# YonghaoHe/LFD-A-Light-and-Fast-Detector

Hardware: NVIDIA H100
Metric: images/sec WIDERFACE-S inference 1280x720 batch=8 per GPU bf16 (higher is better)
Workload: dtype bf16

## Files before the change

### lfd-a-light-and-fast-detector_b200/csrc/conv_umma.cu

```cuda
#include <stdlib.h>

#include <type_traits>

#include "conv_common.cuh"
#include "ptx.cuh"

namespace lfd {

static constexpr int kProdThreads = 128;
static constexpr int kConsumerThreads = 256;
static constexpr int kConvThreads = kConsumerThreads + kProdThreads;

#define LFD_LAMBDA_INLINE __attribute__((always_inline))

#ifdef LFD_B200_TRACE
#define LFD_TRACE(role, idx, slot) \
    do { if (p.trace && blockIdx.x == 0 && (idx) < 32) p.trace[((role) * 32 + (idx)) * 4 + (slot)] = clock64(); } while (0)
#define LFD_TRACE_EPI(tr, idx, slot) \
    do { if ((tr) && blockIdx.x == 0 && (idx) < 16) (tr)[(idx) * 8 + (slot)] = clock64(); } while (0)
#else
#define LFD_TRACE(role, idx, slot) ((void)0)
#define LFD_TRACE_EPI(tr, idx, slot) ((void)0)
#endif

// ... 359 lines not shown
                        store_tile<MODE, COUT, F16>(e, acc3, COUT, bias2, false, false, nullptr, &p.tm_out3, nullptr, c0, c1, n, v0, v1,
                                                    &res_bar[wg], store_count, res_count);
                }
            }
        }
        if (e.wtid == 0) bulk_wait_all();
    } else {
        asm volatile("setmaxnreg.dec.sync.aligned.u32 56;");
        const int ptid = tid - kConsumerThreads;
        if (MODE == MODE_STEM) {
            const bool u8 = p.input_format == 1;
            const int plane = p.H * p.W;
            int rel[kStemPerThread];
            int prc[kStemPerThread];
#pragma unroll
            for (int j = 0; j < kStemPerThread; ++j) {
                const int q = min(ptid + j * kProdThreads, kStemPix - 1);
                const int r = q / kStemCols, c = q - r * kStemCols;
                prc[j] = (r << 8) | c;
                rel[j] = u8 ? (r * p.W + c) * 3 : r * p.W + c;
            }
            const bool last_ok = ptid + (kStemPerThread - 1) * kProdThreads < kStemPix;
            uint32_t raw[kStemPerThread][3];
            uint32_t okmask = 0;
            auto fetch = [&](int tile) LFD_LAMBDA_INLINE {
                const int n = fast_div(tile, p.magic_tpi), t = tile - n * p.tiles_per_img;
                const int ty = fast_div(t, p.magic_tx);
                const int iy0 = 2 * ty * 16 - 1, ix0 = 2 * (t - ty * p.tiles_x) * 8 - 1;
                const bool interior = iy0 >= 0 && ix0 >= 0 && iy0 + kStemRows <= p.H && ix0 + kStemCols <= p.W;
                okmask = 0;
                if (u8) {
                    const uint8_t* img = reinterpret_cast<const uint8_t*>(p.in_raw) + (size_t)n * plane * 3;
                    const uint8_t* org = img + ((ptrdiff_t)iy0 * p.W + ix0) * 3;
#pragma unroll
                    for (int j = 0; j < kStemPerThread; ++j) {
                        if (j == kStemPerThread - 1 && !last_ok) break;
                        const uint8_t* src = org + rel[j];
                        bool ok = true;
                        if (!interior) {
                            const int y = iy0 + (prc[j] >> 8), x = ix0 + (prc[j] & 255);
                            ok = (unsigned)y < (unsigned)p.H && (unsigned)x < (unsigned)p.W;
                            if (!ok) src = img;
                        }
                        okmask |= (ok ? 1u : 0u) << j;
                        raw[j][0] = __ldg(src); raw[j][1] = __ldg(src + 1); raw[j][2] = __ldg(src + 2);
                    }
                } else {
                    const float* img = reinterpret_cast<const float*>(p.in_raw) + (size_t)n * plane * 3;
                    const float* org = img + (ptrdiff_t)iy0 * p.W + ix0;
#pragma unroll
                    for (int j = 0; j < kStemPerThread; ++j) {
                        if (j == kStemPerThread - 1 && !last_ok) break;
                        const float* src = org + rel[j];
                        bool ok = true;
                        if (!interior) {
                            const int y = iy0 + (prc[j] >> 8), x = ix0 + (prc[j] & 255);
                            ok = (unsigned)y < (unsigned)p.H && (unsigned)x < (unsigned)p.W;
                            if (!ok) src = img;
                        }
                        okmask |= (ok ? 1u : 0u) << j;
                        raw[j][0] = __float_as_uint(__ldg(src)); raw[j][1] = __float_as_uint(__ldg(src + plane));
                        raw[j][2] = __float_as_uint(__ldg(src + 2 * plane));
                    }
                }
            };
            uint32_t it = 0;
            pdl_wait();
            if ((int)blockIdx.x < p.num_tiles) fetch(blockIdx.x);
            for (int tile = blockIdx.x; tile < p.num_tiles; tile += gridDim.x, ++it) {
                const uint32_t s = it % SA, ph = (it / SA) & 1;
                if (ptid == 0) LFD_TRACE(0, it, 0);
                mbar_wait(&empty[s], ph ^ 1);
                if (ptid == 0) LFD_TRACE(0, it, 1);
                const uint32_t dst0 = smem_u32(ring) + s * p.stage_bytes + ptid * 8;
#pragma unroll
                for (int j = 0; j < kStemPerThread; ++j) {
                    if (j == kStemPerThread - 1 && !last_ok) break;
                    float f[3];
#pragma unroll
                    for (int k = 0; k < 3; ++k) {
                        f[k] = u8 ? ((float)raw[j][k] - 127.5f) * (1.0f / 127.5f) : __uint_as_float(raw[j][k]);
                        if (!((okmask >> j) & 1u)) f[k] = 0.f;
                    }
                    const uint32_t lo = pack2<F16>(f[0], f[1]), hi = pack2<F16>(f[2], 0.f);
                    asm volatile("st.shared.v2.b32 [%0], {%1, %2};" ::"r"(dst0 + j * (kProdThreads * 8)), "r"(lo), "r"(hi) : "memory");
                }
                fence_proxy_async_smem();
                mbar_arrive(&full[s]);
                if (ptid == 0) LFD_TRACE(0, it, 2);
                if (tile + (int)gridDim.x < p.num_tiles) fetch(tile + gridDim.x);
                if (ptid == 0) LFD_TRACE(0, it, 3);
            }
        } else {
        const int ch = ptid & (cpc - 1);
        const int px0 = ptid >> p.log2_cpc;
        const int pstep = kProd >> p.log2_cpc;
        const uint32_t ch_dst = ch * p.lbo_a;
        const int my_cnt = (p.n_px - px0 + pstep - 1) / pstep;
        uint32_t it = 0;
        pdl_wait();
        for (int tile = blockIdx.x; tile < p.num_tiles; tile += gridDim.x) {
            const int n = fast_div(tile, p.magic_tpi);
            const int t = tile - n * p.tiles_per_img;
            int iy0 = 0, ix0 = 0;
            if (MODE == MODE_FLAT) ix0 = t * 128;
            else {
                const int ty = fast_div(t, p.magic_tx);
                int oy0 = ty * 16, ox0 = (t - ty * p.tiles_x) * 8;
                iy0 = (MODE == MODE_3X3S1) ? oy0 : 2 * oy0;
                ix0 = (MODE == MODE_3X3S1) ? ox0 : 2 * ox0;
            }
            const __nv_bfloat16* img = p.in + (size_t)n * HW * p.Cin + ch * 8;
            constexpr int kDyMin = (MODE == MODE_1X1S2) ? 0 : -1, kDxMin = kDyMin;
            constexpr int kDyMax = (MODE == MODE_3X3S1) ? 16 : ((MODE == MODE_3X3S2) ? 31 : 30);
            constexpr int kDxMax = (MODE == MODE_3X3S1) ? 8 : ((MODE == MODE_3X3S2) ? 15 : 14);
            const bool interior = MODE == MODE_FLAT ? (ix0 + 128 <= HW)
                                                    : (iy0 + kDyMin >= 0 && ix0 + kDxMin >= 0 && iy0 + kDyMax < p.H && ix0 + kDxMax < p.W);
            const __nv_bfloat16* org = img + (ptrdiff_t)(MODE == MODE_FLAT ? ix0 : (iy0 + kDyMin) * p.W + ix0 + kDxMin) * p.Cin;
            for (int cc = 0; cc < n_cc; ++cc, ++it) {
                const uint32_t s = it % SA, ph = (it / SA) & 1;
                if (ptid == 0) LFD_TRACE(0, it, 0);
                mbar_wait(&empty[s], ph ^ 1);
                if (ptid == 0) LFD_TRACE(0, it, 1);
                const uint32_t a_base = smem_u32(ring) + s * p.stage_bytes;
                if (!p.b_resident && ptid == 0) {
                    mbar_arrive_expect_tx(&full[s], p.b_slice_bytes);
                    bulk_g2s(a_base + p.a_stage_bytes, reinterpret_cast<const uint8_t*>(p.w) + (size_t)cc * p.b_slice_bytes,
                             p.b_slice_bytes, &full[s]);
                }
                const __nv_bfloat16* src_cc = img + cc * p.Cc;
                const uint32_t dst_cc = a_base + ch_dst;
                if (MODE == MODE_FLAT) {
                    if (interior) {
                        const __nv_bfloat16* src = org + cc * p.Cc + (size_t)px0 * p.Cin;
                        const size_t sstep = (size_t)pstep * p.Cin;
                        uint32_t dst = dst_cc + px0 * 16;
#pragma unroll 4
                        for (int pxi = px0; pxi < 128; pxi += pstep, src += sstep, dst += pstep * 16) cp_async16_full(dst, src);
                    } else {
#pragma unroll 4
                        for (int pxi = px0; pxi < 128; pxi += pstep) {
                            const int q = ix0 + pxi;
                            const bool ok = q < HW;
                            cp_async16(dst_cc + pxi * 16, src_cc + (ok ? q : 0) * p.Cin, ok);
                        }
                    }
                } else if (interior) {
                    const uint8_t* src = reinterpret_cast<const uint8_t*>(org + cc * p.Cc);
                    const PxEntry* tp = table + px0;
#pragma unroll 4
                    for (int k = 0; k < my_cnt; ++k, tp += pstep) {
                        const uint2 pe = *reinterpret_cast<const uint2*>(tp);
                        cp_async16_full(dst_cc + pe.y, src + pe.x);
                    }
                } else {
#pragma unroll 2
                    for (int pxi = px0; pxi < p.n_px; pxi += pstep) {
                        const PxDelta pd = delta[pxi];
                        const int y = iy0 + pd.dy, x = ix0 + pd.dx;
                        const bool ok = ((unsigned)y < (unsigned)p.H) && ((unsigned)x < (unsigned)p.W);
                        cp_async16(dst_cc + table[pxi].dst_off, src_cc + (ok ? (y * p.W + x) : 0) * p.Cin, ok);
                    }
                }
                cp_async_mbar_arrive(&full[s]);
                if (ptid == 0) LFD_TRACE(0, it, 2);
            }
        }
        cp_async_wait_all();
        }
    }
    LFD_TL_END(p.tl);
}

static constexpr int kS4Rows = 67, kS4Cols = 36, kS4Pix = kS4Rows * kS4Cols;
static constexpr int kS4RowBytes = kS4Cols * 8;
static constexpr int kS4PatchBytes = kS4Pix * 8;
static constexpr int kS4PerThread = (kS4Pix + kProdThreads - 1) / kProdThreads;
static constexpr int kS4Batch = 5;
static constexpr int kS4Groups = kS4Rows * 10;
static constexpr int kS4GroupsPerThread = (kS4Groups + kProdThreads - 1) / kProdThreads;
static constexpr int kS4GroupBatch = 3;
static constexpr int kS4PatchOverrun = 768;
LFD_DEVINL constexpr int s4_slot(int a, int b) {
    return ((a & 1) ? ((b & 1) ? 0 : 147) : ((b & 1) ? 291 : 446)) + (a >> 1) * 9 + (b >> 1);
}
static constexpr int kS4Lbo = 599 * 16;
static constexpr int kS4Bar = 0;
static constexpr int kS4Shift = 256;
static constexpr int kS4Staging = 2048;
static constexpr int kS4W0 = kS4Staging + 2 * 8192;
static constexpr int kS4W1 = kS4W0 + 6144;
static constexpr int kS4W2 = kS4W1 + 8192;
static constexpr int kS4W3 = kS4W2 + 73728;
static constexpr int kS4Planes = kS4W3 + 8192;
static constexpr int kS4Ring = kS4Planes + 8 * kS4Lbo;
static constexpr int kS4Smem = kS4Ring + 2 * kS4PatchBytes + kS4PatchOverrun;
static constexpr int kS4WBytes = kS4Planes - kS4W0;
static_assert(kS4Smem <= 227 * 1024, "stem4 shared memory");

LFD_DEVINL void s4_block(int i, int& a0, int& b0, bool& packed) {
    packed = i == 8 || i == 13;
    a0 = packed ? 32 : 8 * (i < 8 ? i >> 1 : i - 9);
    b0 = i < 8 ? 1 + 8 * (i & 1) : (i == 8 ? 1 : 0);
}
LFD_DEVINL void s4_run(int num_tiles, int& t0, int& t1) {
    t0 = (int)((uint64_t)blockIdx.x * (uint32_t)num_tiles / gridDim.x);
    t1 = (int)((uint64_t)(blockIdx.x + 1) * (uint32_t)num_tiles / gridDim.x);
}

LFD_DEVINL void consumers_bar_sync() { asm volatile("bar.sync 3, 256;" ::: "memory"); }

template <bool F16>
__global__ void __launch_bounds__(kConvThreads, 1) stem4_kernel(const __grid_constant__ UmmaConvParams p) {
    extern __shared__ __align__(1024) uint8_t smem[];
    uint64_t* full = reinterpret_cast<uint64_t*>(smem + kS4Bar);
    uint64_t* empty = full + 2;
    uint64_t* wbar = empty + 2;
    uint64_t* res_bar = wbar + 1;
    float* shifts = reinterpret_cast<float*>(smem + kS4Shift);
    pdl_launch_dependents();
    LFD_TL_BEGIN(p.tl);
    const int tid = threadIdx.x;
    const int warp = tid >> 5;
    const int lane = tid & 31;
    if (tid == 0) {
        for (int i = 0; i < 2; ++i) {
            mbar_init(&full[i], kProdThreads);
            mbar_init(&empty[i], kConsumerThreads / 32);
        }
        mbar_init(wbar, 1);
        mbar_init(&res_bar[0], 1);
        mbar_init(&res_bar[1], 1);
        fence_mbar_init();
    }
    if (tid < 256) {
        const int k = tid >> 6;
        const float* s = k == 0 ? p.shift : (k == 1 ? p.shift2 : (k == 2 ? p.shift_s2 : p.shift_s3));
        shifts[tid] = s ? round16<F16>(s[tid & 63]) : 0.f;
    }
    __syncthreads();

    if (warp < kConsumerThreads / 32) {
        asm volatile("setmaxnreg.inc.sync.aligned.u32 224;");
        const int wg = warp >> 2;
        if (tid == 0) {
            mbar_arrive_expect_tx(wbar, kS4WBytes);
            auto load_w = [&](uint32_t dst, const __nv_bfloat16* src, uint32_t bytes) LFD_LAMBDA_INLINE {
                for (uint32_t off = 0; off < bytes; off += 32768)
                    bulk_g2s(smem_u32(smem) + dst + off, reinterpret_cast<const uint8_t*>(src) + off, bytes - off < 32768 ? bytes - off : 32768, wbar);
            };
            load_w(kS4W0, p.w, kS4W1 - kS4W0);
            load_w(kS4W1, p.w2, kS4W2 - kS4W1);
            load_w(kS4W2, p.w_s2, kS4W3 - kS4W2);
            load_w(kS4W3, p.w_s3, kS4Planes - kS4W3);
        }
        pdl_wait();
        mbar_wait(wbar, 0);

        EpiCtx e;
        e.stg_bytes = 8192u;
        e.nbuf = 1;
        e.stg = smem_u32(smem + kS4Staging) + (uint32_t)wg * 8192u;
        e.r0 = (warp & 3) * 16 + (lane >> 2);
        e.tq = lane & 3;
        e.wtid = tid & 127;
        e.wg = wg;
        e.lane = lane;
#ifdef LFD_B200_TRACE
        e.tr = p.trace && e.wtid == 0 ? p.trace + (3 * 32 + wg) * 4 : nullptr;
#endif
        const float* sh0 = shifts;
        const float* sh1 = shifts + 64;
        const float* sh2 = shifts + 128;
        const float* sh3 = shifts + 192;
        const uint32_t planes = smem_u32(smem + kS4Planes);
        const uint64_t adesc_stem = wgmma_desc(0, 16, 2 * kS4RowBytes);
        const uint64_t adesc_row = wgmma_desc(0, 16, 8 * 16);
        const uint64_t b0desc = wgmma_desc(smem_u32(smem + kS4W0), 64 * 16, 128);
        const uint64_t b1desc = wgmma_desc(smem_u32(smem + kS4W1), 64 * 16, 128);
        const uint64_t b2desc = wgmma_desc(smem_u32(smem + kS4W2), 64 * 16, 128);
        const uint64_t b3desc = wgmma_desc(smem_u32(smem + kS4W3), 64 * 16, 128);
        const uint64_t adesc_pl = wgmma_desc(planes + (uint32_t)wg * 8u * 144u, kS4Lbo, 144);
        const int brow = 2 * (warp & 3), bcol = lane >> 2;
        const int sh = (lane >> 3) & 1, sc = lane & 7;

        int tile0, tile1;
        s4_run(p.num_tiles, tile0, tile1);
        uint32_t store_count = 0, res_count = 0;
        for (int tile = tile0, lt = 0; tile < tile1; ++tile, ++lt) {
            const uint32_t s = lt & 1, ph = (lt >> 1) & 1;
            const int n = fast_div(tile, p.magic_tpi);
            const int t = tile - n * p.tiles_per_img;
            const int ty = fast_div(t, p.magic_tx);
            const int tx = t - ty * p.tiles_x;
            const int oy0 = ty * 16, ox0 = tx * 8;
            const bool inherit = tile > tile0 && tx > 0, pass_on = tile + 1 < tile1 && tx + 1 < p.tiles_x;
            if (e.wtid == 0) LFD_TRACE(1 + wg, lt, 0);
            mbar_wait(&full[s], ph);
            if (e.wtid == 0) LFD_TRACE(1 + wg, lt, 1);
            fence_proxy_async_smem();
            const uint32_t patch = smem_u32(smem + kS4Ring) + s * kS4PatchBytes;

            const int nblk = inherit ? 9 : 14, half = (nblk + 1) >> 1;
            const int first = wg ? half : 0, cnt = wg ? nblk - half : half;
#pragma unroll 1
            for (int kp = 0; kp < (cnt + 1) >> 1; ++kp) {
                int blk[2] = {first + 2 * kp, first + min(2 * kp + 1, cnt - 1)};
                float c0[2][32];
                wgmma_fence_regs<32>(c0[0]);
                wgmma_fence_regs<32>(c0[1]);
                wgmma_fence();
#pragma unroll
                for (int q = 0; q < 2; ++q) {
                    int a0, b0;
                    bool packed;
                    s4_block(blk[q], a0, b0, packed);
                    const uint32_t boff = (uint32_t)(a0 * 2 * kS4RowBytes + b0 * 16);
                    const uint64_t ad = (packed ? adesc_row : adesc_stem) + ((patch + boff) >> 4);
#pragma unroll
                    for (int kh = 0; kh < 3; ++kh)
                        wgmma_ss<64, F16>(c0[q], ad + (uint32_t)(kh * kS4RowBytes / 16), b0desc + (uint32_t)(kh * 2 * 64 * 16 / 16), kh != 0);
                }
                wgmma_commit();
                wgmma_wait<0>();
                wgmma_fence_regs<32>(c0[0]);
                wgmma_fence_regs<32>(c0[1]);
                uint32_t a1[2][16];
#pragma unroll
                for (int q = 0; q < 2; ++q)
#pragma unroll
                    for (int kk = 0; kk < 4; ++kk) {
                        const int c = 16 * kk + 2 * e.tq;
#pragma unroll
                        for (int r = 0; r < 4; ++r) {
                            const float x0 = c0[q][8 * kk + 2 * r] + sh0[c + 8 * (r >> 1)], x1 = c0[q][8 * kk + 2 * r + 1] + sh0[c + 8 * (r >> 1) + 1];
                            a1[q][4 * kk + r] = p.relu ? pack2_relu<F16>(x0, x1) : pack2<F16>(x0, x1);
                        }
                    }
                float c1[2][32];
                wgmma_fence_regs<32>(c1[0]);
                wgmma_fence_regs<32>(c1[1]);
                wgmma_fence();
                tail_mma<64, 64, F16>(c1[0], a1[0], b1desc);
                tail_mma<64, 64, F16>(c1[1], a1[1], b1desc);
                wgmma_commit();
                wgmma_wait<0>();
                wgmma_fence_regs<32>(c1[0]);
                wgmma_fence_regs<32>(c1[1]);
                float2 bv[8];
#pragma unroll
                for (int j = 0; j < 8; ++j) bv[j] = *reinterpret_cast<const float2*>(sh1 + 8 * j + 2 * e.tq);
#pragma unroll
                for (int q = 0; q < 2; ++q) {
                    int a0, b0;
                    bool packed;
                    s4_block(blk[q], a0, b0, packed);
                    if (packed && (warp & 3)) continue;
                    uint32_t v[8][2];
#pragma unroll
                    for (int h = 0; h < 2; ++h) {
                        const int a = packed ? a0 : a0 + brow + h, b = b0 + bcol + (packed ? 8 * h : 0);
                        const int y1 = 2 * oy0 - 1 + a, x1 = 2 * ox0 - 1 + b;
                        const bool in = (unsigned)y1 < (unsigned)p.H1 && (unsigned)x1 < (unsigned)p.W1;
#pragma unroll
                        for (int j = 0; j < 8; ++j) {
                            const float x0 = c1[q][4 * j + 2 * h] + bv[j].x, x1v = c1[q][4 * j + 2 * h + 1] + bv[j].y;
                            const uint32_t w = p.relu2 ? pack2_relu<F16>(x0, x1v) : pack2<F16>(x0, x1v);
                            v[j][h] = in ? w : 0u;
                        }
                    }
                    const int a = packed ? a0 : a0 + brow + sh, b = b0 + sc + (packed ? 8 * sh : 0);
                    const uint32_t addr = planes + (uint32_t)s4_slot(a, b) * 16u + (uint32_t)(lane >> 4) * kS4Lbo;
#pragma unroll
                    for (int k = 0; k < 4; ++k)
                        stmatrix_x4(addr + (uint32_t)(2 * k * kS4Lbo), v[2 * k][0], v[2 * k][1], v[2 * k + 1][0], v[2 * k + 1][1]);
                }
            }
            __syncwarp();
            if (lane == 0) mbar_arrive(&empty[s]);
            if (e.wtid == 0) LFD_TRACE(1 + wg, lt, 2);
            fence_proxy_async_smem();
            consumers_bar_sync();
            if (e.wtid == 0) LFD_TRACE(1 + wg, lt, 3);

            float acc[32];
            wgmma_fence_regs<32>(acc);
            wgmma_fence();
#pragma unroll
            for (int k16 = 0; k16 < 4; ++k16)
#pragma unroll
                for (int tap = 0; tap < 9; ++tap)
                    wgmma_ss<64, F16>(acc, adesc_pl + (uint32_t)(k16 * 2 * kS4Lbo / 16 + s4_slot(tap / 3, tap % 3)),
                                      b2desc + (uint32_t)((tap * 8 + 2 * k16) * 64 * 16 / 16), (k16 | tap) != 0);
            wgmma_commit();
            wgmma_wait<0>();
            wgmma_fence_regs<32>(acc);
            consumers_bar_sync();
            if (pass_on) {
                const int rs = lane >> 3, a = 16 * wg + brow + (rs & 1) + 8 * (rs >> 1);
                const uint32_t src = planes + (uint32_t)(lane & 7) * kS4Lbo + (uint32_t)s4_slot(a, 16) * 16u;
                sts128(src - 8u * 16u, lds128(src));
                if (wg == 1 && brow == 0 && lane < 8) {
                    const uint32_t src32 = planes + (uint32_t)lane * kS4Lbo + (uint32_t)s4_slot(32, 16) * 16u;
                    sts128(src32 - 8u * 16u, lds128(src32));
                }
                __syncwarp();
            }
#ifdef LFD_B200_TRACE
            if (e.wtid == 0 && p.trace && blockIdx.x == 0 && lt < 16) p.trace[(3 * 32 + wg + 2 * lt) * 4 + 3] = clock64();
#endif

            uint32_t a2[16];
#pragma unroll
            for (int kk = 0; kk < 4; ++kk) {
                const int c = 16 * kk + 2 * e.tq;
#pragma unroll
                for (int r = 0; r < 4; ++r) {
                    const float x0 = acc[8 * kk + 2 * r] + sh2[c + 8 * (r >> 1)], x1 = acc[8 * kk + 2 * r + 1] + sh2[c + 8 * (r >> 1) + 1];
                    a2[4 * kk + r] = p.relu_s2 ? pack2_relu<F16>(x0, x1) : pack2<F16>(x0, x1);
                }
            }
            float acc2[32];
            wgmma_fence_regs<32>(acc2);
            wgmma_fence();
            tail_mma<64, 64, F16>(acc2, a2, b3desc);
            wgmma_commit();
            wgmma_wait<0>();
            wgmma_fence_regs<32>(acc2);
            store_tile<MODE_3X3S2, 64, F16>(e, acc2, 64, sh3, (bool)p.relu_s3, false, nullptr, &p.tm_out, &p.tm_res, ox0, oy0 + wg * 8, n,
                                            true, true, &res_bar[wg], store_count, res_count);
        }
        if (e.wtid == 0) bulk_wait_all();
    } else {
        asm volatile("setmaxnreg.dec.sync.aligned.u32 56;");
        const int ptid = tid - kConsumerThreads;
        const bool u8 = p.input_format == 1;
        const int plane = p.H * p.W;
        pdl_wait();
        int tile0, tile1;
        s4_run(p.num_tiles, tile0, tile1);
        for (int tile = tile0, lt = 0; tile < tile1; ++tile, ++lt) {
            const uint32_t s = lt & 1, ph = (lt >> 1) & 1;
            const int n = fast_div(tile, p.magic_tpi), t = tile - n * p.tiles_per_img;
            const int ty = fast_div(t, p.magic_tx);
            const int iy0 = 4 * 16 * ty - 3, ix0 = 4 * 8 * (t - ty * p.tiles_x) - 3;
            const bool interior = iy0 >= 0 && ix0 >= 0 && iy0 + kS4Rows <= p.H && ix0 + kS4Cols <= p.W;
            if (ptid == 0) LFD_TRACE(0, lt, 0);
            mbar_wait(&empty[s], ph ^ 1);
            if (ptid == 0) LFD_TRACE(0, lt, 1);
            const uint32_t dst0 = smem_u32(smem + kS4Ring) + s * kS4PatchBytes;
            if (p.in_words) {
#pragma unroll 1
                for (int j0 = 0; j0 < kS4GroupsPerThread; j0 += kS4GroupBatch) {
                    uint32_t wd[kS4GroupBatch][3];
                    bool ok[kS4GroupBatch];
#pragma unroll
                    for (int j = 0; j < kS4GroupBatch; ++j) {
                        const int q = ptid + (j0 + j) * kProdThreads;
                        const int r = q / 10, g = q - r * 10;
                        const int y = iy0 + r, x = ix0 - 1 + 4 * g;
                        ok[j] = q < kS4Groups && (unsigned)y < (unsigned)p.H && (unsigned)x < (unsigned)p.W;
                        const uint32_t* src = reinterpret_cast<const uint32_t*>(reinterpret_cast<const uint8_t*>(p.in_raw) +
                                                                                ((ptrdiff_t)n * plane + (ptrdiff_t)y * p.W + x) * 3);
#pragma unroll
                        for (int k = 0; k < 3; ++k) wd[j][k] = ok[j] ? __ldg(src + k) : 0u;
                    }
#pragma unroll
                    for (int j = 0; j < kS4GroupBatch; ++j) {
                        const int q = ptid + (j0 + j) * kProdThreads;
                        if (q >= kS4Groups) break;
                        const int r = q / 10, g = q - r * 10;
                        uint32_t px[4][2];
#pragma unroll
                        for (int k = 0; k < 4; ++k) {
                            float f[3];
#pragma unroll
                            for (int c = 0; c < 3; ++c) {
                                const uint32_t byte = (wd[j][(3 * k + c) >> 2] >> (8 * ((3 * k + c) & 3))) & 0xffu;
                                f[c] = ok[j] ? ((float)byte - 127.5f) * (1.0f / 127.5f) : 0.f;
                            }
                            px[k][0] = pack2<F16>(f[0], f[1]);
                            px[k][1] = pack2<F16>(f[2], 0.f);
                        }
                        const uint32_t d = dst0 + (uint32_t)(r * kS4RowBytes + 32 * g);
                        if (g > 0) asm volatile("st.shared.v2.b32 [%0], {%1, %2};" ::"r"(d - 8u), "r"(px[0][0]), "r"(px[0][1]) : "memory");
                        if (g < 9) {
                            asm volatile("st.shared.v4.b32 [%0], {%1, %2, %3, %4};" ::"r"(d), "r"(px[1][0]), "r"(px[1][1]), "r"(px[2][0]),
                                         "r"(px[2][1]) : "memory");
                            asm volatile("st.shared.v2.b32 [%0], {%1, %2};" ::"r"(d + 16u), "r"(px[3][0]), "r"(px[3][1]) : "memory");
                        }
                    }
                }
            } else {
#pragma unroll 1
                for (int j0 = 0; j0 < kS4PerThread; j0 += kS4Batch) {
                    uint32_t raw[kS4Batch][3];
                    bool ok[kS4Batch];
#pragma unroll
                    for (int j = 0; j < kS4Batch; ++j) {
                        const int q = ptid + (j0 + j) * kProdThreads;
                        const int r = q / kS4Cols, c = q - r * kS4Cols;
                        const int y = iy0 + r, x = ix0 + c;
                        ok[j] = q < kS4Pix && (interior || ((unsigned)y < (unsigned)p.H && (unsigned)x < (unsigned)p.W));
                        const ptrdiff_t pix = ok[j] ? (ptrdiff_t)n * plane + (ptrdiff_t)y * p.W + x : 0;
                        if (u8) {
                            const uint8_t* src = reinterpret_cast<const uint8_t*>(p.in_raw) + pix * 3;
                            raw[j][0] = __ldg(src); raw[j][1] = __ldg(src + 1); raw[j][2] = __ldg(src + 2);
                        } else {
                            const float* src = reinterpret_cast<const float*>(p.in_raw) + (ok[j] ? (ptrdiff_t)n * 2 * plane + pix : 0);
                            raw[j][0] = __float_as_uint(__ldg(src)); raw[j][1] = __float_as_uint(__ldg(src + plane));
                            raw[j][2] = __float_as_uint(__ldg(src + 2 * plane));
                        }
                    }
#pragma unroll
                    for (int j = 0; j < kS4Batch; ++j) {
                        const int q = ptid + (j0 + j) * kProdThreads;
                        if (q >= kS4Pix) break;
                        float f[3];
#pragma unroll
                        for (int k = 0; k < 3; ++k) {
                            f[k] = u8 ? ((float)raw[j][k] - 127.5f) * (1.0f / 127.5f) : __uint_as_float(raw[j][k]);
                            if (!ok[j]) f[k] = 0.f;
                        }
                        const uint32_t lo = pack2<F16>(f[0], f[1]), hi = pack2<F16>(f[2], 0.f);
                        asm volatile("st.shared.v2.b32 [%0], {%1, %2};" ::"r"(dst0 + q * 8), "r"(lo), "r"(hi) : "memory");
                    }
                }
            }
            fence_proxy_async_smem();
            mbar_arrive(&full[s]);
            if (ptid == 0) LFD_TRACE(0, lt, 2);
        }
    }
    LFD_TL_END(p.tl);
}

static int configure_with(const ConvGeom& g, int num_sms, int nbuf, UmmaConvParams* out, size_t* smem_bytes, int* grid) {
    UmmaConvParams p;
    memset(&p, 0, sizeof(p));
    p.stg_nbuf = nbuf;
    int mode;
    if (g.stem) {
        if (g.ksize != 3 || g.stride != 2 || g.Cin != 16) return -1;
        mode = MODE_STEM;
    } else if (g.ksize == 1 && g.stride == 1) mode = MODE_FLAT;
    else if (g.ksize == 3 && g.stride == 1) mode = MODE_3X3S1;
    else if (g.ksize == 3 && g.stride == 2) mode = MODE_3X3S2;
    else if (g.ksize == 1 && g.stride == 2) mode = MODE_1X1S2;
    else return -1;
    if (g.Cin % 16 || (g.Cout != 16 && g.Cout != 32 && g.Cout != 64 && g.Cout != 128)) return -1;
    if ((mode == MODE_3X3S1 || mode == MODE_3X3S2) && g.Cout < 32) return -1;
    p.mode = mode;
    p.N = g.N; p.H = g.H; p.W = g.W; p.Cin = g.Cin; p.Ho = g.Ho; p.Wo = g.Wo; p.Cout = g.Cout;
    const int taps = g.stem ? 3 : g.ksize * g.ksize;
    int px_slots;
    if (mode == MODE_FLAT) {
        p.tiles_x = 0; p.tiles_per_img = (g.Ho * g.Wo + 127) / 128;
        p.n_px = 128; px_slots = 128; p.sbo_a = 128;
    } else {
        p.tiles_x = (g.Wo + 7) / 8;
        p.tiles_per_img = p.tiles_x * ((g.Ho + 15) / 16);
        if (mode == MODE_3X3S1) { p.n_px = 180; px_slots = 180; p.sbo_a = 160; }
        else if (mode == MODE_3X3S2) { p.n_px = 561; px_slots = 594; p.sbo_a = 144; }
        else { p.n_px = 128; px_slots = 128; p.sbo_a = 128; }
    }
    const int plane_slots = px_slots | 1;
    p.lbo_a = plane_slots * 16;
    if (mode == MODE_STEM) { p.lbo_a = 16; p.sbo_a = 2 * kStemRowBytes; }
    p.num_tiles = p.tiles_per_img * g.N;
    if (p.num_tiles >= (1 << 24) || p.tiles_per_img >= (1 << 16)) return -5;
    p.magic_tpi = ((1ull << 40) + p.tiles_per_img - 1) / p.tiles_per_img;
    p.magic_tx = p.tiles_x ? ((1ull << 40) + p.tiles_x - 1) / p.tiles_x : 0;
    const int Cf = g.tail_cout > 0 ? g.tail_cout : g.Cout;
    if (g.ds_cout && (mode != MODE_3X3S2 || g.tail_cout || g.ds_cout != g.Cout)) return -6;
    if (g.tail_cout && (g.tail_cout % 16 || g.tail_cout > 128 || g.tail_cout < 16)) return -4;
    const size_t staging = (size_t)nbuf * 128 * Cf * 2;
    size_t hoff = kSmemTableOff;
    p.smem_table_off = (uint32_t)hoff;
    if (mode != MODE_FLAT && mode != MODE_STEM) hoff += ((size_t)p.n_px * 10 + 127) & ~(size_t)127;
    p.smem_bias_off = (uint32_t)hoff; hoff += ((size_t)g.Cout * 4 + 15) & ~(size_t)15;
    p.smem_bias2_off = (uint32_t)hoff; hoff += ((size_t)(g.tail_cout + g.ds_cout) * 4 + 15) & ~(size_t)15;
    p.smem_staging_off = (uint32_t)((hoff + 1023) & ~(size_t)1023);
    const size_t fixed = p.smem_staging_off + staging;
    const size_t w2_bytes = g.tail_cout ? ((size_t)g.Cout * g.tail_cout * 2 + 127) & ~(size_t)127
                                        : (g.ds_cout ? ((size_t)g.Cin * g.ds_cout * 2 + 127) & ~(size_t)127 : 0);
    const size_t post = w2_bytes;
    const size_t budget = 224 * 1024 - post;
    const size_t w_total = (size_t)taps * g.Cin * g.Cout * 2;
    const int cands[3] = {64, 32, 16};
    int best_cc = 0, best_res = 0, best_st = 0;
    auto a_bytes = [&](int cc) -> size_t {
        if (mode == MODE_STEM) return kStemPatchBytes;
        return (((size_t)plane_slots * (cc / 8) * 16) + 127) & ~(size_t)127;
    };
    auto stages_for = [&](int cc, int resident) -> int {
        if (g.Cin % cc) return 0;
        const size_t b_slice = (size_t)taps * cc * g.Cout * 2;
        const size_t stage = a_bytes(cc) + (resident ? 0 : b_slice);
        if (fixed + (resident ? w_total : 0) + 2 * stage > budget) return 0;
        int st = (int)((budget - fixed - (resident ? w_total : 0)) / stage);
        if (st > kMaxStages) st = kMaxStages;
        if (st > 4 && stage >= 8192) st = 4;
        return st;
    };
    static const int force_cc = getenv("LFD_B200_FORCE_CC") ? atoi(getenv("LFD_B200_FORCE_CC")) : 0;
    if (force_cc && mode == MODE_3X3S2) {
        int st = stages_for(force_cc, 1);
        if (st >= 2) { best_cc = force_cc; best_res = 1; best_st = st; }
    }
    for (int pass = 0; pass < 3 && !best_cc; ++pass)
        for (int ci = 0; ci < 3 && !best_cc; ++ci) {
            const int want = pass == 0 ? 3 : 2;
            if (pass < 2 && cands[ci] < 32) continue;
            int st = stages_for(cands[ci], 1);
            if (st >= want) { best_cc = cands[ci]; best_res = 1; best_st = st; }
        }
    if (!best_cc || (best_st < 3 && best_cc < 32)) {
        for (int want = 4; want >= 2; --want) {
            bool found = false;
            for (int ci = 0; ci < 3 && !found; ++ci) {
                int st = stages_for(cands[ci], 0);
                if (st >= want && (!best_cc || st > best_st)) { best_cc = cands[ci]; best_res = 0; best_st = st; found = true; }
            }
            if (found) break;
        }
    }
    if (!best_cc) return -2;
    p.Cc = best_cc; p.b_resident = best_res; p.stages = best_st;
    p.a_stage_bytes = (uint32_t)a_bytes(best_cc);
    p.b_slice_bytes = (uint32_t)((size_t)taps * best_cc * g.Cout * 2);
    p.stage_bytes = p.a_stage_bytes + (best_res ? 0 : p.b_slice_bytes);
    p.w_total_bytes = (uint32_t)w_total;
    p.smem_w_off = (uint32_t)fixed;
    p.smem_ring_off = (uint32_t)(fixed + (best_res ? w_total : 0));
    auto ilog2 = [](int v) { int l = 0; while ((1 << l) < v) ++l; return l; };
    p.log2_cpc = ilog2(p.Cc / 8);
    p.Cf = Cf;
    p.Cout2 = g.tail_cout;
    p.Cout3 = g.ds_cout;
    p.log2_cpr = ilog2(Cf / 8);
    if ((1 << p.log2_cpr) != Cf / 8) return -3;
    size_t off = p.smem_ring_off + (size_t)p.stages * p.stage_bytes;
    p.smem_w2_off = (uint32_t)off; off += w2_bytes;
    *smem_bytes = off;
    *grid = p.num_tiles < num_sms ? p.num_tiles : num_sms;
    *out = p;
    return 0;
}

static int configure_stem4(const ConvGeom& g, int num_sms, UmmaConvParams* out, size_t* smem_bytes, int* grid) {
    if (g.Cin != 3 || g.ksize != 3 || g.stride != 2 || g.Cout != 64 || g.tail_cout != 64 || g.ds_cout) return -1;
    UmmaConvParams p;
    memset(&p, 0, sizeof(p));
    p.mode = MODE_STEM4;
    p.N = g.N; p.H = g.H; p.W = g.W; p.Cin = 3; p.Cout = 64; p.Cout2 = 64; p.Cf = 64;
    p.H1 = (g.H - 1) / 2 + 1; p.W1 = (g.W - 1) / 2 + 1;
    p.Ho = (p.H1 - 1) / 2 + 1; p.Wo = (p.W1 - 1) / 2 + 1;
    if (g.H < 1 || g.W < 1 || g.Ho != p.Ho || g.Wo != p.Wo) return -1;
    p.tiles_x = (p.Wo + 7) / 8;
    p.tiles_per_img = p.tiles_x * ((p.Ho + 15) / 16);
    p.num_tiles = p.tiles_per_img * g.N;
    if (p.num_tiles >= (1 << 24) || p.tiles_per_img >= (1 << 16)) return -5;
    p.magic_tpi = ((1ull << 40) + p.tiles_per_img - 1) / p.tiles_per_img;
    p.magic_tx = ((1ull << 40) + p.tiles_x - 1) / p.tiles_x;
    p.stg_nbuf = 1; p.stages = 2;
    *smem_bytes = kS4Smem;
    *grid = p.num_tiles < num_sms ? p.num_tiles : num_sms;
    *out = p;
    return 0;
}

int umma_conv_configure(const ConvGeom& g, int num_sms, UmmaConvParams* out, size_t* smem_bytes, int* grid) {
    if (g.stem4) return configure_stem4(g, num_sms, out, smem_bytes, grid);
    UmmaConvParams p1, p2;
    size_t s1 = 0, s2 = 0;
    int g1 = 0, g2 = 0;
    const int rc = configure_with(g, num_sms, 1, &p1, &s1, &g1);
    if (rc) return rc;
    if (configure_with(g, num_sms, 2, &p2, &s2, &g2) == 0 && p2.b_resident == p1.b_resident &&
// ... 122 lines not shown
```

Measured before the change: 10250.

## Software-pipeline stem conv blocks and specialize relu/border flags at compile time

```diff
diff --git a/lfd-a-light-and-fast-detector_b200/csrc/conv_umma.cu b/lfd-a-light-and-fast-detector_b200/csrc/conv_umma.cu
--- a/lfd-a-light-and-fast-detector_b200/csrc/conv_umma.cu
+++ b/lfd-a-light-and-fast-detector_b200/csrc/conv_umma.cu
@@ -685,70 +685,55 @@
             const uint32_t patch = smem_u32(smem + kS4Ring) + s * kS4PatchBytes;
 
             const int nblk = inherit ? 9 : 14, half = (nblk + 1) >> 1;
-            const int first = wg ? half : 0, cnt = wg ? nblk - half : half;
-#pragma unroll 1
-            for (int kp = 0; kp < (cnt + 1) >> 1; ++kp) {
-                int blk[2] = {first + 2 * kp, first + min(2 * kp + 1, cnt - 1)};
-                float c0[2][32];
-                wgmma_fence_regs<32>(c0[0]);
-                wgmma_fence_regs<32>(c0[1]);
-                wgmma_fence();
-#pragma unroll
-                for (int q = 0; q < 2; ++q) {
+            const int first = wg ? half : 0, last = wg ? nblk - 1 : half - 1;
+            auto stem01 = [&](auto relu0, auto relu1, auto border) LFD_LAMBDA_INLINE {
+                constexpr bool kRelu0 = decltype(relu0)::value, kRelu1 = decltype(relu1)::value, kBorder = decltype(border)::value;
+                float c0[32], c1[32];
+                uint32_t a1[16];
+                auto stem0_issue = [&](int blk) LFD_LAMBDA_INLINE {
                     int a0, b0;
                     bool packed;
-                    s4_block(blk[q], a0, b0, packed);
+                    s4_block(blk, a0, b0, packed);
                     const uint32_t boff = (uint32_t)(a0 * 2 * kS4RowBytes + b0 * 16);
                     const uint64_t ad = (packed ? adesc_row : adesc_stem) + ((patch + boff) >> 4);
+                    wgmma_fence_regs<32>(c0);
+                    wgmma_fence();
 #pragma unroll
                     for (int kh = 0; kh < 3; ++kh)
-                        wgmma_ss<64, F16>(c0[q], ad + (uint32_t)(kh * kS4RowBytes / 16), b0desc + (uint32_t)(kh * 2 * 64 * 16 / 16), kh != 0);
-                }
-                wgmma_commit();
-                wgmma_wait<0>();
-                wgmma_fence_regs<32>(c0[0]);
-                wgmma_fence_regs<32>(c0[1]);
-                uint32_t a1[2][16];
-#pragma unroll
-                for (int q = 0; q < 2; ++q)
+                        wgmma_ss<64, F16>(c0, ad + (uint32_t)(kh * kS4RowBytes / 16), b0desc + (uint32_t)(kh * 2 * 64 * 16 / 16), kh != 0);
+                    wgmma_commit();
+                };
+                auto stem1_issue = [&]() LFD_LAMBDA_INLINE {
 #pragma unroll
                     for (int kk = 0; kk < 4; ++kk) {
                         const int c = 16 * kk + 2 * e.tq;
 #pragma unroll
                         for (int r = 0; r < 4; ++r) {
-                            const float x0 = c0[q][8 * kk + 2 * r] + sh0[c + 8 * (r >> 1)], x1 = c0[q][8 * kk + 2 * r + 1] + sh0[c + 8 * (r >> 1) + 1];
-                            a1[q][4 * kk + r] = p.relu ? pack2_relu<F16>(x0, x1) : pack2<F16>(x0, x1);
+                            const float x0 = c0[8 * kk + 2 * r] + sh0[c + 8 * (r >> 1)], x1 = c0[8 * kk + 2 * r + 1] + sh0[c + 8 * (r >> 1) + 1];
+                            a1[4 * kk + r] = kRelu0 ? pack2_relu<F16>(x0, x1) : pack2<F16>(x0, x1);
                         }
                     }
-                float c1[2][32];
-                wgmma_fence_regs<32>(c1[0]);
-                wgmma_fence_regs<32>(c1[1]);
-                wgmma_fence();
-                tail_mma<64, 64, F16>(c1[0], a1[0], b1desc);
-                tail_mma<64, 64, F16>(c1[1], a1[1], b1desc);
-                wgmma_commit();
-                wgmma_wait<0>();
-                wgmma_fence_regs<32>(c1[0]);
-                wgmma_fence_regs<32>(c1[1]);
-                float2 bv[8];
-#pragma unroll
-                for (int j = 0; j < 8; ++j) bv[j] = *reinterpret_cast<const float2*>(sh1 + 8 * j + 2 * e.tq);
-#pragma unroll
-                for (int q = 0; q < 2; ++q) {
+                    wgmma_fence_regs<32>(c1);
+                    wgmma_fence();
+                    tail_mma<64, 64, F16>(c1, a1, b1desc);
+                    wgmma_commit();
+                };
+                auto stem1_store = [&](int blk) LFD_LAMBDA_INLINE {
                     int a0, b0;
                     bool packed;
-                    s4_block(blk[q], a0, b0, packed);
-                    if (packed && (warp & 3)) continue;
+                    s4_block(blk, a0, b0, packed);
+                    if (packed && (warp & 3)) return;
                     uint32_t v[8][2];
 #pragma unroll
                     for (int h = 0; h < 2; ++h) {
                         const int a = packed ? a0 : a0 + brow + h, b = b0 + bcol + (packed ? 8 * h : 0);
                         const int y1 = 2 * oy0 - 1 + a, x1 = 2 * ox0 - 1 + b;
-                        const bool in = (unsigned)y1 < (unsigned)p.H1 && (unsigned)x1 < (unsigned)p.W1;
+                        const bool in = !kBorder || ((unsigned)y1 < (unsigned)p.H1 && (unsigned)x1 < (unsigned)p.W1);
 #pragma unroll
                         for (int j = 0; j < 8; ++j) {
-                            const float x0 = c1[q][4 * j + 2 * h] + bv[j].x, x1v = c1[q][4 * j + 2 * h + 1] + bv[j].y;
-                            const uint32_t w = p.relu2 ? pack2_relu<F16>(x0, x1v) : pack2<F16>(x0, x1v);
+                            const float2 bv = *reinterpret_cast<const float2*>(sh1 + 8 * j + 2 * e.tq);
+                            const float x0 = c1[4 * j + 2 * h] + bv.x, x1v = c1[4 * j + 2 * h + 1] + bv.y;
+                            const uint32_t w = kRelu1 ? pack2_relu<F16>(x0, x1v) : pack2<F16>(x0, x1v);
                             v[j][h] = in ? w : 0u;
                         }
                     }
@@ -757,7 +742,37 @@
 #pragma unroll
                     for (int k = 0; k < 4; ++k)
                         stmatrix_x4(addr + (uint32_t)(2 * k * kS4Lbo), v[2 * k][0], v[2 * k][1], v[2 * k + 1][0], v[2 * k + 1][1]);
-                }
+                };
+                stem0_issue(first);
+                wgmma_wait<0>();
+                wgmma_fence_regs<32>(c0);
+#pragma unroll 1
+                for (int blk = first; blk < last; ++blk) {
+                    stem1_issue();
+                    stem0_issue(blk + 1);
+                    wgmma_wait<1>();
+                    wgmma_fence_regs<32>(c1);
+                    stem1_store(blk);
+                    wgmma_wait<0>();
+                    wgmma_fence_regs<32>(c0);
+                }
+                stem1_issue();
+                wgmma_wait<0>();
+                wgmma_fence_regs<32>(c1);
+                stem1_store(last);
+            };
+            const bool border = oy0 == 0 || ox0 == 0 || 2 * oy0 + 31 >= p.H1 || 2 * ox0 + 15 >= p.W1;
+            using T = std::true_type;
+            using F = std::false_type;
+            switch ((p.relu ? 4 : 0) | (p.relu2 ? 2 : 0) | (border ? 1 : 0)) {
+                case 0: stem01(F(), F(), F()); break;
+                case 1: stem01(F(), F(), T()); break;
+                case 2: stem01(F(), T(), F()); break;
+                case 3: stem01(F(), T(), T()); break;
+                case 4: stem01(T(), F(), F()); break;
+                case 5: stem01(T(), F(), T()); break;
+                case 6: stem01(T(), T(), F()); break;
+                default: stem01(T(), T(), T()); break;
             }
             __syncwarp();
             if (lane == 0) mbar_arrive(&empty[s]);
```

New measurement: 10530 (median of 6 runs). 2.8% higher.
